# PaulMayer123/IMS-Toucan-Prosody-Variance

Measured on AMD Instinct MI355X. Metric: mel-frames/sec + vocoder RTF @24kHz, batch=32, 1/2/4/8 MI355X, higher is better.
Workload: dtype bf16

## Files before the change

ims-toucan-prosody-variance_amd/csrc/common.h:

```cpp
#pragma once
#include <hip/hip_runtime.h>
#include <stdint.h>
#include <stdio.h>

#include "../../include/toucan_tts.h"

namespace tts {

void set_error(const char* fmt, ...);

#define TTS_CHECK_ARG(cond, ...)   \
  do {                             \
    if (!(cond)) {                 \
      tts::set_error(__VA_ARGS__); \
      return TTS_E_ARG;            \
    }                              \
  } while (0)

inline int launch_status(const char* what) {
  hipError_t e = hipGetLastError();
  if (e != hipSuccess) {
    set_error("%s: %s", what, hipGetErrorString(e));
    return TTS_E_LAUNCH;
  }
// ... 2 lines not shown

inline hipError_t raise_lds_limit(const void* kernel, unsigned long long& mask) {
  int dev = 0;
  (void)hipGetDevice(&dev);
  const unsigned long long bit = 1ull << (dev & 63);
  if (mask & bit) return hipSuccess;
  int room = 160 * 1024;
  hipFuncAttributes attr;
  if (hipFuncGetAttributes(&attr, kernel) == hipSuccess) room -= (int)attr.sharedSizeBytes;
  else (void)hipGetLastError();
  const hipError_t e = hipFuncSetAttribute(kernel, hipFuncAttributeMaxDynamicSharedMemorySize, room);
  if (e == hipSuccess) mask |= bit;
  else (void)hipGetLastError();
  return e;
}

typedef float f32x16 __attribute__((ext_vector_type(16)));
typedef float f32x4 __attribute__((ext_vector_type(4)));
typedef short bf16x8 __attribute__((ext_vector_type(8)));

__device__ __forceinline__ unsigned short f32_to_bf16(float f) {
  const __bf16 b = (__bf16)f;
  return __builtin_bit_cast(unsigned short, b);
}
__device__ __forceinline__ float bf16_to_f32(unsigned short u) { return __builtin_bit_cast(float, (unsigned int)u << 16); }

typedef _Float16 f16x2 __attribute__((ext_vector_type(2)));
typedef _Float16 f16x8 __attribute__((ext_vector_type(8)));
typedef float f32x2 __attribute__((ext_vector_type(2)));
__device__ __forceinline__ unsigned short f32_to_f16(float f) { return __builtin_bit_cast(unsigned short, (_Float16)f); }
// ... 45 lines not shown
```

ims-toucan-prosody-variance_amd/csrc/pipeline.hip:

```cpp
#include <algorithm>
#include <cmath>
#include <cstdlib>
#include <cstring>
#include <string>
#include <unordered_map>
#include <utility>
#include <vector>

#include "common.h"
#include "../../include/toucan_score.h"

namespace tts {

namespace {

constexpr int ATT = 192, HEADS = 4, DK = 48;

struct Dev {
  void* p = nullptr;
  int64_t shape[4] = {0, 0, 0, 0};
  int ndim = 0, dtype = 0;
  size_t bytes = 0;
};

// ... 409 lines not shown
  b->ff_fused = find(h, p + "ff.fused");
  TTS_TRY(conv_of(h, p + "qkv", &b->qkv));
  TTS_TRY(conv_of(h, p + "out", &b->out));
  TTS_TRY(conv_of(h, p + "pos", &b->pos));
  TTS_TRY(conv_of(h, p + "pw1", &b->pw1));
  TTS_TRY(conv_of(h, p + "pw2", &b->pw2));
  TTS_TRY(fvec(h, p + "u", &b->u));
  TTS_TRY(fvec(h, p + "v", &b->v));
  TTS_TRY(fvec(h, p + "dw_w", &b->dw_w));
  TTS_TRY(fvec(h, p + "dw_b", &b->dw_b));
  return TTS_OK;
}

bool is16(const Handle* h) { return h->cfg.precision == TTS_COMPUTE_BF16 || h->cfg.precision == TTS_COMPUTE_F16; }
int bits16(const Handle* h) { return is16(h) ? 16 : 32; }

int ensure_ptabs(Handle* h, hipStream_t st) {
  const Dev* pe;
  TTS_TRY(need(h, "pe", &pe));
  const int rows = (int)pe->shape[0], pmax = (rows + 1) / 2;
  if (h->pmax == pmax && h->ptab[0]) return TTS_OK;
  TTS_TRY(hip_ok(hipStreamSynchronize(st), "position tables: sync"));
  for (int s = 0; s < 2; ++s) {
    if (h->ptab[s]) (void)hipFree(h->ptab[s]);
    TTS_TRY(hip_ok(hipMalloc(reinterpret_cast<void**>(&h->ptab[s]), (size_t)6 * rows * ATT * sizeof(float)), "position tables: hipMalloc"));
  }
  int one = rows;
  const Layout l = Layout::make(&one, 1, 1);
  for (int s = 0; s < 2; ++s)
    for (int b = 0; b < 6; ++b) {
// ... 79 lines not shown
    } else {
      TTS_TRY(tts_layernorm(x, ATT, ln, ATT, b.ln_g[3], b.ln_b[3], R, ATT, 1e-12f, st));
      TTS_TRY(conv(h, b.ff1, T2(ln, ATT), T2(hid, 1536, b16), l, st, relu));
      TTS_TRY(conv(h, b.ff2, T2(hid, 1536, b16), T2(x, ATT), l, st, half));
      TTS_TRY(tts_layernorm(x, ATT, x, ATT, b.ln_g[4], b.ln_b[4], R, ATT, 1e-12f, st));
    }
  }
  return TTS_OK;
}

size_t conformer_bytes(size_t R) { return R * (ATT * 4 * 4 + 1536 * 4 + 3 * ATT * 4) + 8 * 256; }

size_t phone_arena_bytes(size_t R, size_t B) {
  return conformer_bytes(R) + R * (100 + 3 * ATT + 6 * 256 + 16) * 4 + B * (64 + 2 * ATT + 24 * 256 + 8) * 4 + (1 << 16);
}
size_t frame_arena_bytes(size_t RF) {
  return conformer_bytes(RF) + RF * ((80 + ATT) + 2 * ATT + 3 * 80 + 2 * 256 + ATT + 160 + 4 * ATT + ATT + 8 * ATT + 64) * 4 + (64 << 20);
}
size_t vocoder_stage_bytes(size_t R, int stage, bool fused_mode, bool big) {
  static const int UPS[4] = {8, 48, 192, 384};
  const size_t ch = 256 >> stage, rows = R * UPS[stage], se = fused_mode ? 2 : 4;
  const bool fused = fused_mode && ch <= 128;
  const size_t tensors = 4 + (fused ? 0 : (big ? 3 : 1));
  return tensors * (((rows * ch * se) + 255) & ~(size_t)255) + (1 << 20);
}
size_t vocoder_arena_bytes(size_t R, int arena, bool fused_mode, bool big) {
  size_t m = arena == 1 ? R * 512 * 4 + (1 << 20) : 0;
  for (int i = arena; i < 4; i += 2) m = std::max(m, vocoder_stage_bytes(R, i, fused_mode, big));
  return m;
}
size_t with_growth_slack(size_t bytes) { return bytes + bytes / 8 + (1 << 20); }

// ... 94 lines not shown
  }
  if (dtype == 3) {
    d.p = malloc(std::max<size_t>(d.bytes, 4));
    memcpy(d.p, host, d.bytes);
  } else {
    TTS_TRY(hip_ok(hipMalloc(&d.p, std::max<size_t>(d.bytes, 256)), "tts_load_weights: hipMalloc"));
    TTS_TRY(hip_ok(hipMemcpy(d.p, host, d.bytes, hipMemcpyHostToDevice), "tts_load_weights: upload"));
  }
  h->weights[name] = d;
  return TTS_OK;
}

long long pipeline_workspace_bytes(const Handle* h, int B, int Lmax, int Tmax) {
  if (!h || B <= 0) return 0;
  const size_t RP = (size_t)B * Lmax, RF = (size_t)B * (Tmax + 1);
  size_t total = with_growth_slack(phone_arena_bytes(RP, B)) + with_growth_slack(frame_arena_bytes(RF));
  if (h->cfg.vocoder) {
    const bool fused_mode = is16(h), big = h->cfg.vocoder == 2;
    for (int a = 0; a < 2; ++a) total += with_growth_slack(vocoder_arena_bytes(RF, a, fused_mode, big));
  }
  return (long long)total;
}

long long pipeline_workspace_claimed(const Handle* h) {
  if (!h) return 0;
  return (long long)(h->phone.cap + h->frame.cap + h->voc[0].cap + h->voc[1].cap);
}

int pipeline_encoder(Handle* h, const float* text, const float* utt_emb, const int* lang_ids, const int* phone_lengths, int B,
                     hipStream_t st) {
  TTS_CHECK_ARG(h && text && phone_lengths && B > 0, "tts_encoder: bad arguments");
// ... 101 lines not shown
  const int *pb, *pe;
  TTS_TRY(bounds_of(h, h->lp, st, &pb, &pe));
  TTS_TRY(tts_prosody_control(h->text, 62, h->pitch, h->energy, h->dur, pb, pe, B, duration_scale, pitch_scale, energy_scale, pause_scale, st));
  std::vector<int> d_host(R);
  TTS_TRY(hip_ok(hipMemcpyAsync(d_host.data(), h->dur, (size_t)R * 4, hipMemcpyDeviceToHost, st), "durations to host"));
  TTS_TRY(hip_ok(hipStreamSynchronize(st), "durations to host: sync"));
  h->frames.assign(B, 0);
  for (int u = 0; u < B; ++u) {
    long long t = 0;
    for (int i = 0; i < h->lp.lengths[u]; ++i) t += d_host[h->lp.begins[u] + i];
    h->frames[u] = t > 0 ? (int)t : h->lp.lengths[u];
    if (frames_out) frames_out[u] = h->frames[u];
  }
  h->lf = Layout::make(h->frames.data(), B, 2);
  const size_t RF = h->lf.total;
  TTS_TRY(arena_reserve(h->frame, frame_arena_bytes(RF), st));
  Arena& a = h->frame;
  TTS_ALLOC(cat, a, float, RF * (80 + ATT));
  TTS_TRY(hip_ok(hipMemsetAsync(cat, 0, RF * (80 + ATT) * 4, st), "clear frame buffer"));
  TTS_ALLOC(dec, a, float, RF * ATT);
  h->cat = cat;
  h->dec = dec;
  const float *wp, *bp, *we, *be;
  TTS_TRY(fvec(h, "pitch_w", &wp));
  TTS_TRY(fvec(h, "pitch_b", &bp));
  TTS_TRY(fvec(h, "energy_w", &we));
  TTS_TRY(fvec(h, "energy_b", &be));
  const int *fb, *fe;
  TTS_TRY(bounds_of(h, h->lf, st, &fb, &fe));
  return tts_length_regulate(h->enc, ATT, h->pitch, h->energy, wp, bp, we, be, h->dur, pb, pe, fb, B, h->lf.max_len, h->lp.max_len, ATT,
                             cat + 80, 80 + ATT, dec, ATT, sqrtf((float)ATT), st);
// ... 25 lines not shown
  TTS_TRY(hip_ok(hipStreamSynchronize(st), "durations to host: sync"));
  h->frames.assign(B, 0);
  for (int u = 0; u < B; ++u) {
    long long t = 0;
    for (int i = 0; i < h->lp.lengths[u]; ++i) {
      const int d = d_host[h->lp.begins[u] + i];
      TTS_CHECK_ARG(d >= 0, "tts_teacher_forced: utterance %d, phoneme %d: negative gold duration %d", u, i, d);
      t += d;
    }
    TTS_CHECK_ARG(t <= (1 << 24), "tts_teacher_forced: utterance %d: %lld frames", u, t);
    h->frames[u] = t > 0 ? (int)t : h->lp.lengths[u];
    if (frames_out) frames_out[u] = h->frames[u];
  }
  h->lf = Layout::make(h->frames.data(), B, 2);
  const size_t RF = h->lf.total;
  TTS_TRY(arena_reserve(h->frame, frame_arena_bytes(RF), st));
  Arena& a = h->frame;
  TTS_ALLOC(cat, a, float, RF * (80 + ATT));
  TTS_TRY(hip_ok(hipMemsetAsync(cat, 0, RF * (80 + ATT) * 4, st), "clear frame buffer"));
  TTS_ALLOC(dec, a, float, RF * ATT);
  h->cat = cat;
  h->dec = dec;
  const float *wp, *bp, *we, *be;
  TTS_TRY(fvec(h, "pitch_w", &wp));
  TTS_TRY(fvec(h, "pitch_b", &bp));
  TTS_TRY(fvec(h, "energy_w", &we));
  TTS_TRY(fvec(h, "energy_b", &be));
  const int *pb, *pe, *fb, *fe;
  TTS_TRY(bounds_of(h, h->lp, st, &pb, &pe));
  TTS_TRY(bounds_of(h, h->lf, st, &fb, &fe));
  return tts_length_regulate(h->enc, ATT, h->energy, h->pitch, we, be, wp, bp, h->dur, pb, pe, fb, B, h->lf.max_len, h->lp.max_len, ATT,
// ... 55 lines not shown
  TTS_CHECK_ARG(h && h->mel == h->cat && h->cat, "tts_postflow: run tts_postnet first");
  TTS_CHECK_ARG(z_noise, "tts_postflow: z_noise is required");
  h->split_mode = 1;
  h->tab_which = 0;
  const Layout ls = h->lf.halved();
  const int RF = h->lf.total, RS = RF / 2;
  Arena& a = h->frame;
  const int b16 = bits16(h);
  ConvW gp;
  TTS_TRY(conv_of(h, "g_proj", &gp));
  TTS_ALLOC(g, a, float, (size_t)RF * ATT);
  TTS_TRY(conv(h, gp, T2(h->cat, 80 + ATT), T2(g, ATT), h->lf, st));
  TTS_ALLOC(x, a, float, (size_t)RS * 160);
  TTS_TRY(hip_ok(hipMemcpyAsync(x, z_noise, (size_t)RS * 160 * 4, hipMemcpyDeviceToDevice, st), "flow noise"));
  TTS_ALLOC(hs, a, float, (size_t)RS * 2 * ATT);
  const bool fused = is16(h) && !h->no_fused_wavenet;
  float* hs2 = nullptr;
  TileTab t64;
  if (fused) {
    hs2 = arena_alloc<float>(a, (size_t)RS * 2 * ATT);
    if (!hs2) {
      set_error("tts_postflow: workspace exhausted");
      return TTS_E_ARG;
    }
    TTS_TRY(tiles_of(h, ls, 64, st, &t64));
  }
  TTS_ALLOC(acts, a, char, (size_t)RS * ATT * (b16 / 8));
  TTS_ALLOC(cond, a, float, (size_t)RS * 8 * ATT);
  float* skip = hs + ATT;
  for (int b = 17; b >= 0; --b) {
    const std::string p = "flow." + std::to_string(b) + ".", grp = "flowgrp." + std::to_string(b / 4) + ".";
    ConvW start, end, cnd;
    TTS_TRY(conv_of(h, p + "start", &start));
    TTS_TRY(conv_of(h, p + "end", &end));
    TTS_TRY(conv_of(h, p + "cond", &cnd));
    TTS_TRY(conv(h, start, T2(x, 160), T2(hs, 2 * ATT), ls, st));
    TTS_TRY(conv(h, cnd, T2(g, 2 * ATT), T2(cond, 8 * ATT), ls, st));
    float* cur = hs;
    for (int i = 0; i < 4; ++i) {
      ConvW inl, rs;
      TTS_TRY(conv_of(h, grp + "inl." + std::to_string(i), &inl));
      TTS_TRY(conv_of(h, grp + "res_skip." + std::to_string(i), &rs));
      if (fused) {
        float* nxt = cur == hs ? hs2 : hs;
        TtsWavenetDesc w;
        memset(&w, 0, sizeof(w));
        w.hs_in = cur; w.ld_in = 2 * ATT; w.hs_out = nxt; w.ld_out = 2 * ATT;
        w.cond = cond + (size_t)i * 2 * ATT; w.ld_cond = 8 * ATT;
        w.w1 = inl.w16; w.b1 = inl.bias; w.w2 = rs.w16; w.b2 = rs.bias;
        w.cout2 = rs.cout; w.compute = inl.compute16;
        w.tiles = t64.dev; w.n_tiles = t64.n; w.tile_rows = 64;
        TTS_TRY(tts_wavenet_layer(&w, st));
        cur = nxt;
        continue;
      }
      ConvOpt oi;
      oi.preadd = cond + (size_t)i * 2 * ATT;
      oi.ld_preadd = 8 * ATT;
      TTS_TRY(conv(h, inl, T2(hs, 2 * ATT), T2(acts, ATT, b16), ls, st, oi));
      ConvOpt orr;
      orr.accumulate = true;
      TTS_TRY(conv(h, rs, T2(acts, ATT, b16), i < 3 ? T2(hs, 2 * ATT) : T2(skip, 2 * ATT), ls, st, orr));
    }
    ConvOpt oe;
    oe.aux = x + 80;
    oe.ld_aux = 160;
    oe.fp32_only = true;
// ... 374 lines not shown
```

ims-toucan-prosody-variance_amd/csrc/wavenet.hip:

```cpp
#include "common.h"

namespace tts {

namespace {
constexpr int WN_H = 192;
constexpr int WN_BM = 64;
constexpr int WN_TAPS = 5;
constexpr int WN_XP = WN_H + 8;
constexpr int WN_KS = 32;
constexpr int WN_SLAB_BYTES = (WN_KS / 8) * 384 * 16;
constexpr int WN_SLABS1 = WN_TAPS * (WN_H / WN_KS);
constexpr int WN_SLABS2 = WN_H / WN_KS;
constexpr int WN_RING = 5;
constexpr int WN_LOADS = 6;
}

template <bool F16>
__global__ __launch_bounds__(256) void wavenet_layer_kernel(const TtsWavenetDesc d) {
  extern __shared__ __attribute__((aligned(16))) unsigned char lds_raw[];
  unsigned short* xs = reinterpret_cast<unsigned short*>(lds_raw);
  unsigned char* ring = lds_raw + ((WN_BM + WN_TAPS - 1) * WN_XP * 2 + 255) / 256 * 256;
  const TtsTile tile = d.tiles[blockIdx.x];
  const int tid = threadIdx.x, lane = tid & 63, wave = tid >> 6, wm = wave >> 1, wn = wave & 1, lrow = lane & 31, lk = lane >> 5;
  const int n2 = d.cout2;
  const int units2 = (WN_KS / 8) * n2;
  const int total = WN_SLABS1 + WN_SLABS2;
  const char* w1 = reinterpret_cast<const char*>(d.w1);
  const char* w2 = reinterpret_cast<const char*>(d.w2);

  auto issue_piece = [&](int s, int i) __attribute__((always_inline)) {
    if (s >= total) return;
    const bool second = s >= WN_SLABS1;
    const int units = second ? units2 : (WN_KS / 8) * 384;
    const char* src = second ? w2 + (size_t)(s - WN_SLABS1) * units2 * 16 : w1 + (size_t)s * WN_SLAB_BYTES;
    unsigned char* dst = ring + (size_t)(s % WN_RING) * WN_SLAB_BYTES;
#ifdef WN_DIAG_NO_DMA
    if (s >= WN_RING) return;
#endif
    const int u0 = i * 256 + wave * 64;
    int u = u0 + lane;
    u = u < units ? u : units - 1;
    __builtin_amdgcn_global_load_lds((const void __attribute__((address_space(1)))*)(src + (size_t)u * 16),
                                     (void __attribute__((address_space(3)))*)(dst + (size_t)u0 * 16), 16, 0, 0);
  };
  auto issue = [&](int s) __attribute__((always_inline)) {
#pragma unroll
    for (int i = 0; i < WN_LOADS; ++i) issue_piece(s, i);
  };

#pragma unroll
  for (int i = 0; i < WN_RING - 1; ++i) issue(i);
  {
    constexpr int Q4 = WN_H / 4, ROWS = WN_BM + WN_TAPS - 1, TOTAL = ROWS * Q4, PER = 7;
    for (int base = tid; base < TOTAL; base += 256 * PER) {
      float4 v[PER];
#pragma unroll
      for (int p = 0; p < PER; ++p) {
        int e = base + p * 256;
        e = e < TOTAL ? e : TOTAL - 1;
        const int r = e / Q4, c4 = (e % Q4) * 4;
        const int gr = tile.row0 - 2 + r;
        const int grc = gr < tile.seq_begin ? tile.seq_begin : (gr >= tile.seq_end ? tile.seq_end - 1 : gr);
        v[p] = *reinterpret_cast<const float4*>(d.hs_in + (size_t)grc * d.ld_in + c4);
        if (gr != grc) v[p] = make_float4(0.f, 0.f, 0.f, 0.f);
      }
#pragma unroll
      for (int p = 0; p < PER; ++p) {
        const int e = base + p * 256;
        if (e < TOTAL) {
          const int r = e / Q4, c4 = (e % Q4) * 4;
          *reinterpret_cast<uint2*>(xs + r * WN_XP + c4) = make_uint2(pack16<F16>(v[p].x, v[p].y), pack16<F16>(v[p].z, v[p].w));
        }
      }
    }
  }
  f32x16 acc[6];
#pragma unroll
  for (int j = 0; j < 6; ++j)
#pragma unroll
    for (int r = 0; r < 16; ++r) acc[j][r] = 0.0f;

  auto wait_for = [&](int s) __attribute__((always_inline)) {
    const int behind = total - 1 - s;
    static_assert(WN_RING >= 3 && WN_RING <= 6, "one wait per number of slabs in flight below");
    if (WN_RING >= 6 && behind >= 4) asm volatile("s_waitcnt vmcnt(%0)" ::"n"(4 * WN_LOADS) : "memory");
    else if (WN_RING >= 5 && behind >= 3) asm volatile("s_waitcnt vmcnt(%0)" ::"n"(3 * WN_LOADS) : "memory");
    else if (WN_RING >= 4 && behind >= 2) asm volatile("s_waitcnt vmcnt(%0)" ::"n"(2 * WN_LOADS) : "memory");
    else if (behind >= 1) asm volatile("s_waitcnt vmcnt(%0)" ::"n"(WN_LOADS) : "memory");
    else asm volatile("s_waitcnt vmcnt(0)" ::: "memory");
    asm volatile("s_waitcnt lgkmcnt(0)" ::: "memory");
    __builtin_amdgcn_s_barrier();
  };

  for (int s = 0; s < WN_SLABS1; ++s) {
    wait_for(s);
    const int tap = s / (WN_H / WN_KS), k0 = (s % (WN_H / WN_KS)) * WN_KS;
    const unsigned short* wb = reinterpret_cast<const unsigned short*>(ring + (size_t)(s % WN_RING) * WN_SLAB_BYTES);
    bf16x8 xf[WN_KS / 16], wf[WN_KS / 16][6];
#pragma unroll
    for (int kk = 0; kk < WN_KS / 16; ++kk) {
      xf[kk] = *reinterpret_cast<const bf16x8*>(xs + (wm * 32 + lrow + tap) * WN_XP + k0 + kk * 16 + lk * 8);
#pragma unroll
      for (int j = 0; j < 6; ++j) {
        const int col = (j < 3 ? 0 : WN_H) + wn * 96 + (j % 3) * 32 + lrow;
        wf[kk][j] = *reinterpret_cast<const bf16x8*>(wb + ((size_t)(kk * 2 + lk) * 384 + col) * 8);
      }
    }
    __builtin_amdgcn_sched_barrier(0);
#ifndef WN_DIAG_NO_MFMA
#pragma unroll
    for (int kk = 0; kk < WN_KS / 16; ++kk)
#pragma unroll
      for (int j = 0; j < 6; ++j) {
        if ((kk * 6 + j) % 2 == 0) {
          issue_piece(s + WN_RING - 1, (kk * 6 + j) / 2);
          __builtin_amdgcn_sched_barrier(0);
        }
        acc[j] = mfma16<F16>(wf[kk][j], xf[kk], acc[j]);
      }
#else
    issue(s + WN_RING - 1);
    for (int j = 0; j < 6; ++j) acc[j][0] += bf16_to_f32(wf[0][j][0]) + bf16_to_f32(xf[1][1]) + bf16_to_f32(wf[1][j][2]);
#endif
    __builtin_amdgcn_sched_barrier(0);
  }
  __builtin_amdgcn_s_barrier();
  {
    const int t = wm * 32 + lrow, row = tile.row0 + t;
    const bool live = row < tile.seq_end;
    const float* cr = d.cond + (size_t)(live ? row : tile.seq_end - 1) * d.ld_cond;
#pragma unroll
    for (int j = 0; j < 3; ++j) {
#pragma unroll
      for (int rq = 0; rq < 4; ++rq) {
        const int c = wn * 96 + j * 32 + 8 * rq + 4 * lk;
        const float4 ba = *reinterpret_cast<const float4*>(d.b1 + c), bg = *reinterpret_cast<const float4*>(d.b1 + WN_H + c);
        const float4 ca = *reinterpret_cast<const float4*>(cr + c), cg = *reinterpret_cast<const float4*>(cr + WN_H + c);
        const float av[4] = {acc[j][4 * rq] + ba.x + ca.x, acc[j][4 * rq + 1] + ba.y + ca.y, acc[j][4 * rq + 2] + ba.z + ca.z, acc[j][4 * rq + 3] + ba.w + ca.w};
        const float gv[4] = {acc[j + 3][4 * rq] + bg.x + cg.x, acc[j + 3][4 * rq + 1] + bg.y + cg.y, acc[j + 3][4 * rq + 2] + bg.z + cg.z,
                             acc[j + 3][4 * rq + 3] + bg.w + cg.w};
        float v[4];
#pragma unroll
        for (int q = 0; q < 4; ++q) {
          const float th = 2.0f * __builtin_amdgcn_rcpf(1.0f + __expf(-2.0f * av[q])) - 1.0f;
          v[q] = th * __builtin_amdgcn_rcpf(1.0f + __expf(-gv[q]));
        }
        *reinterpret_cast<uint2*>(xs + t * WN_XP + c) = make_uint2(pack16<F16>(v[0], v[1]), pack16<F16>(v[2], v[3]));
      }
    }
#pragma unroll
    for (int j = 0; j < 6; ++j)
#pragma unroll
      for (int r = 0; r < 16; ++r) acc[j][r] = 0.0f;
  }
  const int half2 = n2 >> 1, nj = n2 >> 6;
  for (int s = WN_SLABS1; s < total; ++s) {
    wait_for(s);
    const int k0 = (s - WN_SLABS1) * WN_KS;
    const unsigned short* wb = reinterpret_cast<const unsigned short*>(ring + (size_t)(s % WN_RING) * WN_SLAB_BYTES);
    bf16x8 xf[WN_KS / 16], wf[WN_KS / 16][6];
#pragma unroll
    for (int kk = 0; kk < WN_KS / 16; ++kk) {
      xf[kk] = *reinterpret_cast<const bf16x8*>(xs + (wm * 32 + lrow) * WN_XP + k0 + kk * 16 + lk * 8);
#pragma unroll
      for (int j = 0; j < 6; ++j) {
        const int col = wn * half2 + (j < nj ? j : 0) * 32 + lrow;
        wf[kk][j] = *reinterpret_cast<const bf16x8*>(wb + ((size_t)(kk * 2 + lk) * n2 + col) * 8);
      }
    }
    __builtin_amdgcn_sched_barrier(0);
#pragma unroll
    for (int kk = 0; kk < WN_KS / 16; ++kk)
#pragma unroll
      for (int j = 0; j < 6; ++j) {
        if ((kk * 6 + j) % 2 == 0) {
          issue_piece(s + WN_RING - 1, (kk * 6 + j) / 2);
          __builtin_amdgcn_sched_barrier(0);
        }
        if (j < nj) acc[j] = mfma16<F16>(wf[kk][j], xf[kk], acc[j]);
      }
    __builtin_amdgcn_sched_barrier(0);
  }
  {
    const int row = tile.row0 + wm * 32 + lrow;
    if (row < tile.seq_end) {
      const int col0 = n2 == 384 ? 0 : WN_H;
      const float* ir = d.hs_in + (size_t)row * d.ld_in + col0;
      float* orow = d.hs_out + (size_t)row * d.ld_out + col0;
#pragma unroll
      for (int j = 0; j < 6; ++j) {
        if (j < nj) {
#pragma unroll
          for (int rq = 0; rq < 4; ++rq) {
            const int c = wn * half2 + j * 32 + 8 * rq + 4 * lk;
            const float4 b = *reinterpret_cast<const float4*>(d.b2 + c), x = *reinterpret_cast<const float4*>(ir + c);
            *reinterpret_cast<float4*>(orow + c) = make_float4((acc[j][4 * rq] + b.x) + x.x, (acc[j][4 * rq + 1] + b.y) + x.y,
                                                               (acc[j][4 * rq + 2] + b.z) + x.z, (acc[j][4 * rq + 3] + b.w) + x.w);
          }
        }
      }
    }
  }
}

int wavenet_layer(const TtsWavenetDesc& d, hipStream_t st) {
  TTS_CHECK_ARG(d.hs_in && d.hs_out && d.cond && d.w1 && d.b1 && d.w2 && d.b2 && d.tiles, "wavenet_layer: null pointer");
  TTS_CHECK_ARG(d.hs_in != d.hs_out, "wavenet_layer: the hidden state cannot be updated in place (the 5-tap conv reads neighbouring tiles)");
  TTS_CHECK_ARG(d.cout2 == 384 || d.cout2 == 192, "wavenet_layer: res/skip width %d (384, or 192 for the last layer)", d.cout2);
  TTS_CHECK_ARG(d.compute == TTS_COMPUTE_BF16 || d.compute == TTS_COMPUTE_F16, "wavenet_layer: 16-bit MFMA configurations only (compute %d)", d.compute);
  TTS_CHECK_ARG(d.tile_rows == WN_BM, "wavenet_layer: tile table must use %d rows, got %d", WN_BM, d.tile_rows);
  TTS_CHECK_ARG((d.ld_in & 3) == 0 && (d.ld_out & 3) == 0 && (d.ld_cond & 3) == 0 && ((uintptr_t)d.hs_in & 15) == 0 && ((uintptr_t)d.hs_out & 15) == 0 &&
                    ((uintptr_t)d.cond & 15) == 0 && ((uintptr_t)d.w1 & 15) == 0 && ((uintptr_t)d.w2 & 15) == 0 && ((uintptr_t)d.b1 & 15) == 0 &&
                    ((uintptr_t)d.b2 & 15) == 0,
                "wavenet_layer: rows and weights must be 16-byte aligned");
  if (d.n_tiles == 0) return TTS_OK;
  const size_t lds = ((size_t)(WN_BM + WN_TAPS - 1) * WN_XP * 2 + 255) / 256 * 256 + WN_RING * (size_t)WN_SLAB_BYTES;
  static unsigned long long raised[2] = {0, 0};
  const bool f16 = d.compute == TTS_COMPUTE_F16;
  const void* k = f16 ? reinterpret_cast<const void*>(wavenet_layer_kernel<true>) : reinterpret_cast<const void*>(wavenet_layer_kernel<false>);
  if (raise_lds_limit(k, raised[f16 ? 1 : 0]) != hipSuccess) {
    set_error("wavenet_layer: raising the dynamic LDS limit failed");
    return TTS_E_LAUNCH;
  }
  if (f16) hipLaunchKernelGGL(wavenet_layer_kernel<true>, dim3(d.n_tiles), dim3(256), lds, st, d);
  else hipLaunchKernelGGL(wavenet_layer_kernel<false>, dim3(d.n_tiles), dim3(256), lds, st, d);
  return launch_status("wavenet_layer");
}

}

extern "C" int tts_wavenet_layer(const TtsWavenetDesc* d, tts_stream_t stream) {
  if (!d) {
    tts::set_error("tts_wavenet_layer: null descriptor");
    return TTS_E_ARG;
  }
  return tts::wavenet_layer(*d, reinterpret_cast<hipStream_t>(stream));
}
```

Baseline: 562,300.

## Fuse flow conditioning projection into wavenet layer kernel and stream weights through registers

The postflow conditioning conv (384 -> 1536) is no longer run as a separate GEMM into a large cond buffer. Each wavenet layer kernel now loads the g rows into LDS and computes its own 384-column slice of the conditioning projection alongside the dilated conv. The weight pipeline also changes, from an LDS ring fed by global_load_lds to per-wave register prefetching with a depth-4 global_load_dwordx4 queue and a different wave-to-tile mapping. This saves a launch and the write and read of the cond tensor and shrinks the frame arena, at the cost of extra per-layer MFMA work and higher register pressure.

Measured after the change: 576,600, median of 6. 1.03x the previous value.

```diff
diff --git a/ims-toucan-prosody-variance_amd/csrc/common.h b/ims-toucan-prosody-variance_amd/csrc/common.h
--- a/ims-toucan-prosody-variance_amd/csrc/common.h
+++ b/ims-toucan-prosody-variance_amd/csrc/common.h
@@ -40,6 +40,16 @@
   else (void)hipGetLastError();
   return e;
 }
+
+struct WavenetCond {
+  const float* g;
+  int ld_g;
+  const void* wc;
+  int wc_n;
+  int col0;
+  const float* bc;
+};
+int wavenet_layer_cond(const TtsWavenetDesc& d, const WavenetCond& c, hipStream_t st);
 
 typedef float f32x16 __attribute__((ext_vector_type(16)));
 typedef float f32x4 __attribute__((ext_vector_type(4)));
diff --git a/ims-toucan-prosody-variance_amd/csrc/pipeline.hip b/ims-toucan-prosody-variance_amd/csrc/pipeline.hip
--- a/ims-toucan-prosody-variance_amd/csrc/pipeline.hip
+++ b/ims-toucan-prosody-variance_amd/csrc/pipeline.hip
@@ -447,6 +447,7 @@
 
 bool is16(const Handle* h) { return h->cfg.precision == TTS_COMPUTE_BF16 || h->cfg.precision == TTS_COMPUTE_F16; }
 int bits16(const Handle* h) { return is16(h) ? 16 : 32; }
+bool postflow_cond_buffer(const Handle* h) { return !is16(h) || h->no_fused_wavenet; }
 
 int ensure_ptabs(Handle* h, hipStream_t st) {
   const Dev* pe;
@@ -556,8 +557,8 @@
 size_t phone_arena_bytes(size_t R, size_t B) {
   return conformer_bytes(R) + R * (100 + 3 * ATT + 6 * 256 + 16) * 4 + B * (64 + 2 * ATT + 24 * 256 + 8) * 4 + (1 << 16);
 }
-size_t frame_arena_bytes(size_t RF) {
-  return conformer_bytes(RF) + RF * ((80 + ATT) + 2 * ATT + 3 * 80 + 2 * 256 + ATT + 160 + 4 * ATT + ATT + 8 * ATT + 64) * 4 + (64 << 20);
+size_t frame_arena_bytes(size_t RF, bool cond_buffer) {
+  return conformer_bytes(RF) + RF * ((80 + ATT) + 2 * ATT + 3 * 80 + 2 * 256 + ATT + 160 + 4 * ATT + ATT + (cond_buffer ? 8 * ATT : 0) + 64) * 4 + (64 << 20);
 }
 size_t vocoder_stage_bytes(size_t R, int stage, bool fused_mode, bool big) {
   static const int UPS[4] = {8, 48, 192, 384};
@@ -682,7 +683,7 @@
 long long pipeline_workspace_bytes(const Handle* h, int B, int Lmax, int Tmax) {
   if (!h || B <= 0) return 0;
   const size_t RP = (size_t)B * Lmax, RF = (size_t)B * (Tmax + 1);
-  size_t total = with_growth_slack(phone_arena_bytes(RP, B)) + with_growth_slack(frame_arena_bytes(RF));
+  size_t total = with_growth_slack(phone_arena_bytes(RP, B)) + with_growth_slack(frame_arena_bytes(RF, postflow_cond_buffer(h)));
   if (h->cfg.vocoder) {
     const bool fused_mode = is16(h), big = h->cfg.vocoder == 2;
     for (int a = 0; a < 2; ++a) total += with_growth_slack(vocoder_arena_bytes(RF, a, fused_mode, big));
@@ -814,7 +815,7 @@
   }
   h->lf = Layout::make(h->frames.data(), B, 2);
   const size_t RF = h->lf.total;
-  TTS_TRY(arena_reserve(h->frame, frame_arena_bytes(RF), st));
+  TTS_TRY(arena_reserve(h->frame, frame_arena_bytes(RF, postflow_cond_buffer(h)), st));
   Arena& a = h->frame;
   TTS_ALLOC(cat, a, float, RF * (80 + ATT));
   TTS_TRY(hip_ok(hipMemsetAsync(cat, 0, RF * (80 + ATT) * 4, st), "clear frame buffer"));
@@ -870,7 +871,7 @@
   }
   h->lf = Layout::make(h->frames.data(), B, 2);
   const size_t RF = h->lf.total;
-  TTS_TRY(arena_reserve(h->frame, frame_arena_bytes(RF), st));
+  TTS_TRY(arena_reserve(h->frame, frame_arena_bytes(RF, postflow_cond_buffer(h)), st));
   Arena& a = h->frame;
   TTS_ALLOC(cat, a, float, RF * (80 + ATT));
   TTS_TRY(hip_ok(hipMemsetAsync(cat, 0, RF * (80 + ATT) * 4, st), "clear frame buffer"));
@@ -956,7 +957,7 @@
   TTS_ALLOC(x, a, float, (size_t)RS * 160);
   TTS_TRY(hip_ok(hipMemcpyAsync(x, z_noise, (size_t)RS * 160 * 4, hipMemcpyDeviceToDevice, st), "flow noise"));
   TTS_ALLOC(hs, a, float, (size_t)RS * 2 * ATT);
-  const bool fused = is16(h) && !h->no_fused_wavenet;
+  const bool fused = !postflow_cond_buffer(h);
   float* hs2 = nullptr;
   TileTab t64;
   if (fused) {
@@ -967,9 +968,19 @@
     }
     TTS_TRY(tiles_of(h, ls, 64, st, &t64));
   }
-  TTS_ALLOC(acts, a, char, (size_t)RS * ATT * (b16 / 8));
-  TTS_ALLOC(cond, a, float, (size_t)RS * 8 * ATT);
+  char* acts = nullptr;
+  float* cond = nullptr;
+  if (!fused) {
+    acts = arena_alloc<char>(a, (size_t)RS * ATT * (b16 / 8));
+    cond = arena_alloc<float>(a, (size_t)RS * 8 * ATT);
+    if (!acts || !cond) {
+      set_error("tts_postflow: workspace exhausted");
+      return TTS_E_ARG;
+    }
+  }
   float* skip = hs + ATT;
+  double live_rows = 0;
+  for (int n : ls.lengths) live_rows += n;
   for (int b = 17; b >= 0; --b) {
     const std::string p = "flow." + std::to_string(b) + ".", grp = "flowgrp." + std::to_string(b / 4) + ".";
     ConvW start, end, cnd;
@@ -977,7 +988,7 @@
     TTS_TRY(conv_of(h, p + "end", &end));
     TTS_TRY(conv_of(h, p + "cond", &cnd));
     TTS_TRY(conv(h, start, T2(x, 160), T2(hs, 2 * ATT), ls, st));
-    TTS_TRY(conv(h, cnd, T2(g, 2 * ATT), T2(cond, 8 * ATT), ls, st));
+    if (!fused) TTS_TRY(conv(h, cnd, T2(g, 2 * ATT), T2(cond, 8 * ATT), ls, st));
     float* cur = hs;
     for (int i = 0; i < 4; ++i) {
       ConvW inl, rs;
@@ -988,11 +999,21 @@
         TtsWavenetDesc w;
         memset(&w, 0, sizeof(w));
         w.hs_in = cur; w.ld_in = 2 * ATT; w.hs_out = nxt; w.ld_out = 2 * ATT;
-        w.cond = cond + (size_t)i * 2 * ATT; w.ld_cond = 8 * ATT;
         w.w1 = inl.w16; w.b1 = inl.bias; w.w2 = rs.w16; w.b2 = rs.bias;
         w.cout2 = rs.cout; w.compute = inl.compute16;
         w.tiles = t64.dev; w.n_tiles = t64.n; w.tile_rows = 64;
-        TTS_TRY(tts_wavenet_layer(&w, st));
+        TTS_CHECK_ARG(cnd.w16 && cnd.mode == TTS_MODE_LINEAR && cnd.compute16 == inl.compute16 && cnd.cin == 2 * ATT && cnd.cin_pad == 2 * ATT && cnd.cout == 8 * ATT &&
+                          cnd.taps == 1 && cnd.wn >= 8 * ATT,
+                      "tts_postflow: %scond is not a 16-bit 1-tap 384 -> 1536 conv", p.c_str());
+        const WavenetCond wc = {g, 2 * ATT, cnd.w16, cnd.wn, i * 2 * ATT, cnd.bias};
+        ProfRec* pr = nullptr;
+        if (h->prof_on && prof_wants(h, "wavenet_layer"))
+          pr = prof_open(h, "wavenet_layer", 2.0 * live_rows * (ATT * 5 * 2 * ATT + 2 * ATT * 2 * ATT + (double)ATT * rs.cout),
+                         live_rows * 4.0 * (2 * ATT + rs.cout + 2 * ATT) + 2.0 * (5 * ATT * 2 * ATT + 2 * ATT * 2 * ATT + ATT * rs.cout),
+                         live_rows * rs.cout, st);
+        const int rc = wavenet_layer_cond(w, wc, st);
+        if (pr) (void)hipEventRecord(pr->e1, st);
+        TTS_TRY(rc);
         cur = nxt;
         continue;
       }
diff --git a/ims-toucan-prosody-variance_amd/csrc/wavenet.hip b/ims-toucan-prosody-variance_amd/csrc/wavenet.hip
--- a/ims-toucan-prosody-variance_amd/csrc/wavenet.hip
+++ b/ims-toucan-prosody-variance_amd/csrc/wavenet.hip
@@ -7,49 +7,83 @@
 constexpr int WN_BM = 64;
 constexpr int WN_TAPS = 5;
 constexpr int WN_XP = WN_H + 8;
-constexpr int WN_KS = 32;
-constexpr int WN_SLAB_BYTES = (WN_KS / 8) * 384 * 16;
-constexpr int WN_SLABS1 = WN_TAPS * (WN_H / WN_KS);
-constexpr int WN_SLABS2 = WN_H / WN_KS;
-constexpr int WN_RING = 5;
-constexpr int WN_LOADS = 6;
-}
-
-template <bool F16>
-__global__ __launch_bounds__(256) void wavenet_layer_kernel(const TtsWavenetDesc d) {
+constexpr int WN_G = 2 * WN_H;
+constexpr int WN_GP = WN_G + 8;
+constexpr int WN_STEPS1 = WN_TAPS * (WN_H / 16);
+constexpr int WN_STEPSC = WN_G / 16;
+constexpr int WN_STEPS2 = WN_H / 16;
+constexpr int WN_DEPTH = 4;
+constexpr int WN_L = 4;
+constexpr size_t WN_XS_BYTES = ((size_t)(WN_BM + WN_TAPS - 1) * WN_XP * 2 + 255) / 256 * 256;
+constexpr size_t WN_GS_BYTES = (size_t)WN_BM * WN_GP * 2;
+static_assert(WN_STEPS1 % WN_DEPTH == 0 && WN_STEPSC % WN_DEPTH == 0 && WN_STEPS2 % WN_DEPTH == 0 && (WN_H / 16) % WN_DEPTH == 0,
+              "a block of WN_DEPTH k-steps stays inside one tap and one product");
+}
+
+template <bool F16, bool FUSED>
+__global__ __launch_bounds__(256) void wavenet_layer_kernel(const TtsWavenetDesc d, const WavenetCond cd) {
   extern __shared__ __attribute__((aligned(16))) unsigned char lds_raw[];
   unsigned short* xs = reinterpret_cast<unsigned short*>(lds_raw);
-  unsigned char* ring = lds_raw + ((WN_BM + WN_TAPS - 1) * WN_XP * 2 + 255) / 256 * 256;
+  unsigned short* gs = reinterpret_cast<unsigned short*>(lds_raw + WN_XS_BYTES);
   const TtsTile tile = d.tiles[blockIdx.x];
-  const int tid = threadIdx.x, lane = tid & 63, wave = tid >> 6, wm = wave >> 1, wn = wave & 1, lrow = lane & 31, lk = lane >> 5;
+  const int tid = threadIdx.x, lane = tid & 63, lrow = lane & 31, lk = lane >> 5;
+  const int wave = __builtin_amdgcn_readfirstlane(tid >> 6);
+  const int P0 = (wave * 5 + 1) / 3, P1 = wave < 2 ? 1 : 4, fP = wave & 1, fQ = fP ^ 1;
   const int n2 = d.cout2;
-  const int units2 = (WN_KS / 8) * n2;
-  const int total = WN_SLABS1 + WN_SLABS2;
-  const char* w1 = reinterpret_cast<const char*>(d.w1);
-  const char* w2 = reinterpret_cast<const char*>(d.w2);
-
-  auto issue_piece = [&](int s, int i) __attribute__((always_inline)) {
-    if (s >= total) return;
-    const bool second = s >= WN_SLABS1;
-    const int units = second ? units2 : (WN_KS / 8) * 384;
-    const char* src = second ? w2 + (size_t)(s - WN_SLABS1) * units2 * 16 : w1 + (size_t)s * WN_SLAB_BYTES;
-    unsigned char* dst = ring + (size_t)(s % WN_RING) * WN_SLAB_BYTES;
-#ifdef WN_DIAG_NO_DMA
-    if (s >= WN_RING) return;
-#endif
-    const int u0 = i * 256 + wave * 64;
-    int u = u0 + lane;
-    u = u < units ? u : units - 1;
-    __builtin_amdgcn_global_load_lds((const void __attribute__((address_space(1)))*)(src + (size_t)u * 16),
-                                     (void __attribute__((address_space(3)))*)(dst + (size_t)u0 * 16), 16, 0, 0);
-  };
-  auto issue = [&](int s) __attribute__((always_inline)) {
-#pragma unroll
-    for (int i = 0; i < WN_LOADS; ++i) issue_piece(s, i);
-  };
-
-#pragma unroll
-  for (int i = 0; i < WN_RING - 1; ++i) issue(i);
+  const int cb0 = n2 == 384 ? 3 * wave : P0, cb1 = n2 == 384 ? 3 * wave + 1 : P1, cb2 = n2 == 384 ? 3 * wave + 2 : P1;
+
+  typedef unsigned int u32x4 __attribute__((ext_vector_type(4)));
+#define WN_GLOAD128(dst_, ptr_) asm volatile("global_load_dwordx4 %0, %1, off" : "=v"(dst_) : "v"(ptr_) : "memory")
+#define WN_WAIT_VM(n_) asm volatile("s_waitcnt vmcnt(%0)" ::"n"(n_) : "memory")
+#define WN_PIN(r_) asm volatile("" : "+v"(r_))
+  u32x4 wr[WN_DEPTH][WN_L];
+  const char *q0, *q1, *q2, *q3;
+  size_t qs;
+  auto request = [&](int slot) __attribute__((always_inline)) {
+    WN_GLOAD128(wr[slot][0], q0);
+    WN_GLOAD128(wr[slot][1], q1);
+    WN_GLOAD128(wr[slot][2], q2);
+    WN_GLOAD128(wr[slot][3], q3);
+    q0 += qs; q1 += qs; q2 += qs; q3 += qs;
+  };
+  auto arrive = [&](int slot) __attribute__((always_inline)) {
+    WN_WAIT_VM((WN_DEPTH - 1) * WN_L);
+    WN_PIN(wr[slot][0]);
+    WN_PIN(wr[slot][1]);
+    WN_PIN(wr[slot][2]);
+    WN_PIN(wr[slot][3]);
+  };
+  auto stream_pairs = [&](const void* w, int n, int col0) __attribute__((always_inline)) {
+    const char* b = reinterpret_cast<const char*>(w) + ((size_t)lk * n + col0 + lrow) * 16;
+    q0 = b + P0 * 512; q1 = q0 + WN_H * 16; q2 = b + P1 * 512; q3 = q2 + WN_H * 16;
+    qs = (size_t)n * 32;
+  };
+  auto stream_res_skip = [&]() __attribute__((always_inline)) {
+    const char* b = reinterpret_cast<const char*>(d.w2) + ((size_t)lk * n2 + lrow) * 16;
+    q0 = b + cb0 * 512; q1 = b + cb1 * 512; q2 = b + cb2 * 512; q3 = q2;
+    qs = (size_t)n2 * 32;
+  };
+  auto publish = [&]() __attribute__((always_inline)) {
+    asm volatile("s_waitcnt lgkmcnt(0)" ::: "memory");
+    __builtin_amdgcn_s_barrier();
+  };
+
+  constexpr int GQ4 = WN_G / 4, GPER = WN_BM * GQ4 / 256;
+  f32x4 gv[FUSED ? GPER : 1];
+  if constexpr (FUSED) {
+#pragma unroll
+    for (int p = 0; p < GPER; ++p) {
+      const int e = tid + p * 256, r = e / GQ4, c4 = (e % GQ4) * 4;
+      int gr = tile.row0 + r;
+      gr = gr < tile.seq_end ? gr : tile.seq_end - 1;
+      const float* gp = cd.g + (size_t)gr * cd.ld_g + c4;
+      asm volatile("global_load_dwordx4 %0, %1, off" : "=a"(gv[p]) : "v"(gp) : "memory");
+    }
+  }
+  stream_pairs(d.w1, 2 * WN_H, 0);
+#pragma unroll
+  for (int u = 0; u < WN_DEPTH; ++u) request(u);
+
   {
     constexpr int Q4 = WN_H / 4, ROWS = WN_BM + WN_TAPS - 1, TOTAL = ROWS * Q4, PER = 7;
     for (int base = tid; base < TOTAL; base += 256 * PER) {
@@ -74,158 +108,223 @@
       }
     }
   }
-  f32x16 acc[6];
+  publish();
+
+  f32x16 acc[6], accc[FUSED ? 6 : 1];
 #pragma unroll
   for (int j = 0; j < 6; ++j)
 #pragma unroll
     for (int r = 0; r < 16; ++r) acc[j][r] = 0.0f;
 
-  auto wait_for = [&](int s) __attribute__((always_inline)) {
-    const int behind = total - 1 - s;
-    static_assert(WN_RING >= 3 && WN_RING <= 6, "one wait per number of slabs in flight below");
-    if (WN_RING >= 6 && behind >= 4) asm volatile("s_waitcnt vmcnt(%0)" ::"n"(4 * WN_LOADS) : "memory");
-    else if (WN_RING >= 5 && behind >= 3) asm volatile("s_waitcnt vmcnt(%0)" ::"n"(3 * WN_LOADS) : "memory");
-    else if (WN_RING >= 4 && behind >= 2) asm volatile("s_waitcnt vmcnt(%0)" ::"n"(2 * WN_LOADS) : "memory");
-    else if (behind >= 1) asm volatile("s_waitcnt vmcnt(%0)" ::"n"(WN_LOADS) : "memory");
-    else asm volatile("s_waitcnt vmcnt(0)" ::: "memory");
-    asm volatile("s_waitcnt lgkmcnt(0)" ::: "memory");
-    __builtin_amdgcn_s_barrier();
-  };
-
-  for (int s = 0; s < WN_SLABS1; ++s) {
-    wait_for(s);
-    const int tap = s / (WN_H / WN_KS), k0 = (s % (WN_H / WN_KS)) * WN_KS;
-    const unsigned short* wb = reinterpret_cast<const unsigned short*>(ring + (size_t)(s % WN_RING) * WN_SLAB_BYTES);
-    bf16x8 xf[WN_KS / 16], wf[WN_KS / 16][6];
-#pragma unroll
-    for (int kk = 0; kk < WN_KS / 16; ++kk) {
-      xf[kk] = *reinterpret_cast<const bf16x8*>(xs + (wm * 32 + lrow + tap) * WN_XP + k0 + kk * 16 + lk * 8);
-#pragma unroll
-      for (int j = 0; j < 6; ++j) {
-        const int col = (j < 3 ? 0 : WN_H) + wn * 96 + (j % 3) * 32 + lrow;
-        wf[kk][j] = *reinterpret_cast<const bf16x8*>(wb + ((size_t)(kk * 2 + lk) * 384 + col) * 8);
-      }
-    }
-    __builtin_amdgcn_sched_barrier(0);
-#ifndef WN_DIAG_NO_MFMA
-#pragma unroll
-    for (int kk = 0; kk < WN_KS / 16; ++kk)
-#pragma unroll
-      for (int j = 0; j < 6; ++j) {
-        if ((kk * 6 + j) % 2 == 0) {
-          issue_piece(s + WN_RING - 1, (kk * 6 + j) / 2);
-          __builtin_amdgcn_sched_barrier(0);
+  auto xload = [&](bf16x8& xP, bf16x8& xQ, const unsigned short* xrow, int pitch) __attribute__((always_inline)) {
+    xP = *reinterpret_cast<const bf16x8*>(xrow + (fP * 32 + lrow) * pitch + lk * 8);
+    xQ = *reinterpret_cast<const bf16x8*>(xrow + (fQ * 32 + lrow) * pitch + lk * 8);
+  };
+  auto pair_step = [&](int slot, f32x16 (&a)[6], bf16x8& xP, bf16x8& xQ, const unsigned short* xnext, int pitch) __attribute__((always_inline)) {
+    const bf16x8 cP = xP, cQ = xQ;
+    xload(xP, xQ, xnext, pitch);
+    arrive(slot);
+    u32x4 wf[WN_L];
+#pragma unroll
+    for (int i = 0; i < WN_L; ++i) wf[i] = wr[slot][i];
+    a[0] = mfma16<F16>(__builtin_bit_cast(bf16x8, wf[0]), cP, a[0]);
+    a[1] = mfma16<F16>(__builtin_bit_cast(bf16x8, wf[0]), cQ, a[1]);
+    a[2] = mfma16<F16>(__builtin_bit_cast(bf16x8, wf[1]), cP, a[2]);
+    a[3] = mfma16<F16>(__builtin_bit_cast(bf16x8, wf[1]), cQ, a[3]);
+    a[4] = mfma16<F16>(__builtin_bit_cast(bf16x8, wf[2]), cP, a[4]);
+    a[5] = mfma16<F16>(__builtin_bit_cast(bf16x8, wf[3]), cP, a[5]);
+    request(slot);
+  };
+  bf16x8 xP, xQ;
+  auto window_at = [&](int s) __attribute__((always_inline)) {
+    s = s < WN_STEPS1 ? s : WN_STEPS1 - 1;
+    return xs + (s / (WN_H / 16)) * WN_XP + (s % (WN_H / 16)) * 16;
+  };
+
+  xload(xP, xQ, window_at(0), WN_XP);
+#pragma unroll 1
+  for (int base = 0; base < WN_STEPS1; base += WN_DEPTH) {
+    if (base == WN_STEPS1 - WN_DEPTH) {
+      if constexpr (FUSED) stream_pairs(cd.wc, cd.wc_n, cd.col0);
+      else stream_res_skip();
+    }
+#pragma unroll
+    for (int u = 0; u < WN_DEPTH; ++u) pair_step(u, acc, xP, xQ, window_at(base + u + 1), WN_XP);
+  }
+  if constexpr (FUSED) {
+#pragma unroll
+    for (int p = 0; p < GPER; ++p) {
+      asm volatile("" : "+a"(gv[p]));
+      const int e = tid + p * 256, r = e / GQ4, c4 = (e % GQ4) * 4;
+      *reinterpret_cast<uint2*>(gs + r * WN_GP + c4) = make_uint2(pack16<F16>(gv[p][0], gv[p][1]), pack16<F16>(gv[p][2], gv[p][3]));
+    }
+  }
+  publish();
+  if constexpr (FUSED) {
+#pragma unroll
+    for (int j = 0; j < 6; ++j)
+#pragma unroll
+      for (int r = 0; r < 16; ++r) accc[j][r] = 0.0f;
+    xload(xP, xQ, gs, WN_GP);
+#pragma unroll 1
+    for (int base = 0; base < WN_STEPSC; base += WN_DEPTH) {
+      if (base == WN_STEPSC - WN_DEPTH) stream_res_skip();
+#pragma unroll
+      for (int u = 0; u < WN_DEPTH; ++u) {
+        const int s1 = base + u + 1 < WN_STEPSC ? base + u + 1 : WN_STEPSC - 1;
+        pair_step(u, accc, xP, xQ, gs + s1 * 16, WN_GP);
+      }
+    }
+  }
+  {
+    auto gate = [&](const f32x16& aa, const f32x16& ag, const f32x16& ca, const f32x16& cg, int pb, int f) __attribute__((always_inline)) {
+      const int t = f * 32 + lrow, row = tile.row0 + t;
+      const float* cr = FUSED ? nullptr : d.cond + (size_t)(row < tile.seq_end ? row : tile.seq_end - 1) * d.ld_cond;
+#pragma unroll
+      for (int rq = 0; rq < 4; ++rq) {
+        const int c = pb * 32 + 8 * rq + 4 * lk;
+        const float4 ba = *reinterpret_cast<const float4*>(d.b1 + c), bg = *reinterpret_cast<const float4*>(d.b1 + WN_H + c);
+        float pa[4], pg[4];
+        if constexpr (FUSED) {
+          const float4 ea = *reinterpret_cast<const float4*>(cd.bc + cd.col0 + c), eg = *reinterpret_cast<const float4*>(cd.bc + cd.col0 + WN_H + c);
+          const float eav[4] = {ea.x, ea.y, ea.z, ea.w}, egv[4] = {eg.x, eg.y, eg.z, eg.w};
+#pragma unroll
+          for (int q = 0; q < 4; ++q) {
+            pa[q] = (ca[4 * rq + q] + eav[q]) + 0.0f;
+            pg[q] = (cg[4 * rq + q] + egv[q]) + 0.0f;
+          }
+        } else {
+          const float4 ea = *reinterpret_cast<const float4*>(cr + c), eg = *reinterpret_cast<const float4*>(cr + WN_H + c);
+          pa[0] = ea.x; pa[1] = ea.y; pa[2] = ea.z; pa[3] = ea.w;
+          pg[0] = eg.x; pg[1] = eg.y; pg[2] = eg.z; pg[3] = eg.w;
         }
-        acc[j] = mfma16<F16>(wf[kk][j], xf[kk], acc[j]);
-      }
-#else
-    issue(s + WN_RING - 1);
-    for (int j = 0; j < 6; ++j) acc[j][0] += bf16_to_f32(wf[0][j][0]) + bf16_to_f32(xf[1][1]) + bf16_to_f32(wf[1][j][2]);
-#endif
-    __builtin_amdgcn_sched_barrier(0);
-  }
-  __builtin_amdgcn_s_barrier();
-  {
-    const int t = wm * 32 + lrow, row = tile.row0 + t;
-    const bool live = row < tile.seq_end;
-    const float* cr = d.cond + (size_t)(live ? row : tile.seq_end - 1) * d.ld_cond;
-#pragma unroll
-    for (int j = 0; j < 3; ++j) {
-#pragma unroll
-      for (int rq = 0; rq < 4; ++rq) {
-        const int c = wn * 96 + j * 32 + 8 * rq + 4 * lk;
-        const float4 ba = *reinterpret_cast<const float4*>(d.b1 + c), bg = *reinterpret_cast<const float4*>(d.b1 + WN_H + c);
-        const float4 ca = *reinterpret_cast<const float4*>(cr + c), cg = *reinterpret_cast<const float4*>(cr + WN_H + c);
-        const float av[4] = {acc[j][4 * rq] + ba.x + ca.x, acc[j][4 * rq + 1] + ba.y + ca.y, acc[j][4 * rq + 2] + ba.z + ca.z, acc[j][4 * rq + 3] + ba.w + ca.w};
-        const float gv[4] = {acc[j + 3][4 * rq] + bg.x + cg.x, acc[j + 3][4 * rq + 1] + bg.y + cg.y, acc[j + 3][4 * rq + 2] + bg.z + cg.z,
-                             acc[j + 3][4 * rq + 3] + bg.w + cg.w};
+        const float bav[4] = {ba.x, ba.y, ba.z, ba.w}, bgv[4] = {bg.x, bg.y, bg.z, bg.w};
         float v[4];
 #pragma unroll
         for (int q = 0; q < 4; ++q) {
-          const float th = 2.0f * __builtin_amdgcn_rcpf(1.0f + __expf(-2.0f * av[q])) - 1.0f;
-          v[q] = th * __builtin_amdgcn_rcpf(1.0f + __expf(-gv[q]));
+          const float av = aa[4 * rq + q] + bav[q] + pa[q], gvv = ag[4 * rq + q] + bgv[q] + pg[q];
+          const float th = 2.0f * __builtin_amdgcn_rcpf(1.0f + __expf(-2.0f * av)) - 1.0f;
+          v[q] = th * __builtin_amdgcn_rcpf(1.0f + __expf(-gvv));
         }
         *reinterpret_cast<uint2*>(xs + t * WN_XP + c) = make_uint2(pack16<F16>(v[0], v[1]), pack16<F16>(v[2], v[3]));
       }
-    }
+    };
+    constexpr int CZ = FUSED ? 1 : 0;
+    gate(acc[0], acc[2], accc[0 * CZ], accc[2 * CZ], P0, fP);
+    gate(acc[1], acc[3], accc[1 * CZ], accc[3 * CZ], P0, fQ);
+    gate(acc[4], acc[5], accc[4 * CZ], accc[5 * CZ], P1, fP);
 #pragma unroll
     for (int j = 0; j < 6; ++j)
 #pragma unroll
       for (int r = 0; r < 16; ++r) acc[j][r] = 0.0f;
   }
-  const int half2 = n2 >> 1, nj = n2 >> 6;
-  for (int s = WN_SLABS1; s < total; ++s) {
-    wait_for(s);
-    const int k0 = (s - WN_SLABS1) * WN_KS;
-    const unsigned short* wb = reinterpret_cast<const unsigned short*>(ring + (size_t)(s % WN_RING) * WN_SLAB_BYTES);
-    bf16x8 xf[WN_KS / 16], wf[WN_KS / 16][6];
-#pragma unroll
-    for (int kk = 0; kk < WN_KS / 16; ++kk) {
-      xf[kk] = *reinterpret_cast<const bf16x8*>(xs + (wm * 32 + lrow) * WN_XP + k0 + kk * 16 + lk * 8);
-#pragma unroll
-      for (int j = 0; j < 6; ++j) {
-        const int col = wn * half2 + (j < nj ? j : 0) * 32 + lrow;
-        wf[kk][j] = *reinterpret_cast<const bf16x8*>(wb + ((size_t)(kk * 2 + lk) * n2 + col) * 8);
-      }
-    }
-    __builtin_amdgcn_sched_barrier(0);
-#pragma unroll
-    for (int kk = 0; kk < WN_KS / 16; ++kk)
-#pragma unroll
-      for (int j = 0; j < 6; ++j) {
-        if ((kk * 6 + j) % 2 == 0) {
-          issue_piece(s + WN_RING - 1, (kk * 6 + j) / 2);
-          __builtin_amdgcn_sched_barrier(0);
-        }
-        if (j < nj) acc[j] = mfma16<F16>(wf[kk][j], xf[kk], acc[j]);
-      }
-    __builtin_amdgcn_sched_barrier(0);
+  publish();
+  xload(xP, xQ, xs, WN_XP);
+#pragma unroll 1
+  for (int base = 0; base < WN_STEPS2; base += WN_DEPTH) {
+    if (base == WN_STEPS2 - WN_DEPTH) {
+      q0 -= qs; q1 -= qs; q2 -= qs; q3 -= qs;
+      qs = 0;
+    }
+#pragma unroll
+    for (int u = 0; u < WN_DEPTH; ++u) {
+      const bf16x8 cP = xP, cQ = xQ;
+      const int s1 = base + u + 1 < WN_STEPS2 ? base + u + 1 : WN_STEPS2 - 1;
+      xload(xP, xQ, xs + s1 * 16, WN_XP);
+      arrive(u);
+      u32x4 wf[3];
+#pragma unroll
+      for (int i = 0; i < 3; ++i) wf[i] = wr[u][i];
+      acc[0] = mfma16<F16>(__builtin_bit_cast(bf16x8, wf[0]), cP, acc[0]);
+      acc[1] = mfma16<F16>(__builtin_bit_cast(bf16x8, wf[0]), cQ, acc[1]);
+      acc[2] = mfma16<F16>(__builtin_bit_cast(bf16x8, wf[1]), cP, acc[2]);
+      if (n2 == 384) {
+        acc[3] = mfma16<F16>(__builtin_bit_cast(bf16x8, wf[1]), cQ, acc[3]);
+        acc[4] = mfma16<F16>(__builtin_bit_cast(bf16x8, wf[2]), cP, acc[4]);
+        acc[5] = mfma16<F16>(__builtin_bit_cast(bf16x8, wf[2]), cQ, acc[5]);
+      }
+      request(u);
+    }
+  }
+  WN_WAIT_VM(0);
+#pragma unroll
+  for (int u = 0; u < WN_DEPTH; ++u) {
+    WN_PIN(wr[u][0]);
+    WN_PIN(wr[u][1]);
+    WN_PIN(wr[u][2]);
+    WN_PIN(wr[u][3]);
   }
   {
-    const int row = tile.row0 + wm * 32 + lrow;
-    if (row < tile.seq_end) {
-      const int col0 = n2 == 384 ? 0 : WN_H;
+    const int col0 = n2 == 384 ? 0 : WN_H;
+    auto store_block = [&](const f32x16& a, int cb, int f) __attribute__((always_inline)) {
+      const int row = tile.row0 + f * 32 + lrow;
+      if (row >= tile.seq_end) return;
       const float* ir = d.hs_in + (size_t)row * d.ld_in + col0;
       float* orow = d.hs_out + (size_t)row * d.ld_out + col0;
 #pragma unroll
-      for (int j = 0; j < 6; ++j) {
-        if (j < nj) {
-#pragma unroll
-          for (int rq = 0; rq < 4; ++rq) {
-            const int c = wn * half2 + j * 32 + 8 * rq + 4 * lk;
-            const float4 b = *reinterpret_cast<const float4*>(d.b2 + c), x = *reinterpret_cast<const float4*>(ir + c);
-            *reinterpret_cast<float4*>(orow + c) = make_float4((acc[j][4 * rq] + b.x) + x.x, (acc[j][4 * rq + 1] + b.y) + x.y,
-                                                               (acc[j][4 * rq + 2] + b.z) + x.z, (acc[j][4 * rq + 3] + b.w) + x.w);
-          }
-        }
-      }
-    }
-  }
-}
-
-int wavenet_layer(const TtsWavenetDesc& d, hipStream_t st) {
-  TTS_CHECK_ARG(d.hs_in && d.hs_out && d.cond && d.w1 && d.b1 && d.w2 && d.b2 && d.tiles, "wavenet_layer: null pointer");
+      for (int rq = 0; rq < 4; ++rq) {
+        const int c = cb * 32 + 8 * rq + 4 * lk;
+        const float4 b = *reinterpret_cast<const float4*>(d.b2 + c), x = *reinterpret_cast<const float4*>(ir + c);
+        *reinterpret_cast<float4*>(orow + c) = make_float4((a[4 * rq] + b.x) + x.x, (a[4 * rq + 1] + b.y) + x.y, (a[4 * rq + 2] + b.z) + x.z, (a[4 * rq + 3] + b.w) + x.w);
+      }
+    };
+    store_block(acc[0], cb0, fP);
+    store_block(acc[1], cb0, fQ);
+    store_block(acc[2], cb1, fP);
+    if (n2 == 384) {
+      store_block(acc[3], cb1, fQ);
+      store_block(acc[4], cb2, fP);
+      store_block(acc[5], cb2, fQ);
+    }
+  }
+#undef WN_GLOAD128
+#undef WN_WAIT_VM
+#undef WN_PIN
+}
+
+namespace {
+int wavenet_launch(const TtsWavenetDesc& d, const WavenetCond* c, hipStream_t st) {
+  TTS_CHECK_ARG(d.hs_in && d.hs_out && d.w1 && d.b1 && d.w2 && d.b2 && d.tiles, "wavenet_layer: null pointer");
   TTS_CHECK_ARG(d.hs_in != d.hs_out, "wavenet_layer: the hidden state cannot be updated in place (the 5-tap conv reads neighbouring tiles)");
   TTS_CHECK_ARG(d.cout2 == 384 || d.cout2 == 192, "wavenet_layer: res/skip width %d (384, or 192 for the last layer)", d.cout2);
   TTS_CHECK_ARG(d.compute == TTS_COMPUTE_BF16 || d.compute == TTS_COMPUTE_F16, "wavenet_layer: 16-bit MFMA configurations only (compute %d)", d.compute);
   TTS_CHECK_ARG(d.tile_rows == WN_BM, "wavenet_layer: tile table must use %d rows, got %d", WN_BM, d.tile_rows);
-  TTS_CHECK_ARG((d.ld_in & 3) == 0 && (d.ld_out & 3) == 0 && (d.ld_cond & 3) == 0 && ((uintptr_t)d.hs_in & 15) == 0 && ((uintptr_t)d.hs_out & 15) == 0 &&
-                    ((uintptr_t)d.cond & 15) == 0 && ((uintptr_t)d.w1 & 15) == 0 && ((uintptr_t)d.w2 & 15) == 0 && ((uintptr_t)d.b1 & 15) == 0 &&
-                    ((uintptr_t)d.b2 & 15) == 0,
+  TTS_CHECK_ARG((d.ld_in & 3) == 0 && (d.ld_out & 3) == 0 && ((uintptr_t)d.hs_in & 15) == 0 && ((uintptr_t)d.hs_out & 15) == 0 && ((uintptr_t)d.w1 & 15) == 0 &&
+                    ((uintptr_t)d.w2 & 15) == 0 && ((uintptr_t)d.b1 & 15) == 0 && ((uintptr_t)d.b2 & 15) == 0,
                 "wavenet_layer: rows and weights must be 16-byte aligned");
+  if (c) {
+    TTS_CHECK_ARG(c->g && c->wc && c->bc, "wavenet_layer: null conditioning pointer");
+    TTS_CHECK_ARG(c->ld_g >= WN_G && (c->ld_g & 3) == 0 && c->col0 >= 0 && (c->col0 & 31) == 0 && c->col0 + 2 * WN_H <= c->wc_n,
+                  "wavenet_layer: conditioning columns %d .. of %d, row stride %d", c->col0, c->wc_n, c->ld_g);
+    TTS_CHECK_ARG(((uintptr_t)c->g & 15) == 0 && ((uintptr_t)c->wc & 15) == 0 && ((uintptr_t)c->bc & 15) == 0, "wavenet_layer: conditioning operands must be 16-byte aligned");
+  } else {
+    TTS_CHECK_ARG(d.cond, "wavenet_layer: null pointer");
+    TTS_CHECK_ARG((d.ld_cond & 3) == 0 && ((uintptr_t)d.cond & 15) == 0, "wavenet_layer: rows and weights must be 16-byte aligned");
+  }
   if (d.n_tiles == 0) return TTS_OK;
-  const size_t lds = ((size_t)(WN_BM + WN_TAPS - 1) * WN_XP * 2 + 255) / 256 * 256 + WN_RING * (size_t)WN_SLAB_BYTES;
-  static unsigned long long raised[2] = {0, 0};
   const bool f16 = d.compute == TTS_COMPUTE_F16;
-  const void* k = f16 ? reinterpret_cast<const void*>(wavenet_layer_kernel<true>) : reinterpret_cast<const void*>(wavenet_layer_kernel<false>);
-  if (raise_lds_limit(k, raised[f16 ? 1 : 0]) != hipSuccess) {
-    set_error("wavenet_layer: raising the dynamic LDS limit failed");
-    return TTS_E_LAUNCH;
-  }
-  if (f16) hipLaunchKernelGGL(wavenet_layer_kernel<true>, dim3(d.n_tiles), dim3(256), lds, st, d);
-  else hipLaunchKernelGGL(wavenet_layer_kernel<false>, dim3(d.n_tiles), dim3(256), lds, st, d);
+  const WavenetCond none = {nullptr, 0, nullptr, 0, 0, nullptr};
+  if (c) {
+    const size_t lds = WN_XS_BYTES + WN_GS_BYTES;
+    static unsigned long long raised[2] = {0, 0};
+    const void* k = f16 ? reinterpret_cast<const void*>(wavenet_layer_kernel<true, true>) : reinterpret_cast<const void*>(wavenet_layer_kernel<false, true>);
+    if (raise_lds_limit(k, raised[f16 ? 1 : 0]) != hipSuccess) {
+      set_error("wavenet_layer: raising the dynamic LDS limit failed");
+      return TTS_E_LAUNCH;
+    }
+    if (f16) hipLaunchKernelGGL((wavenet_layer_kernel<true, true>), dim3(d.n_tiles), dim3(256), lds, st, d, *c);
+    else hipLaunchKernelGGL((wavenet_layer_kernel<false, true>), dim3(d.n_tiles), dim3(256), lds, st, d, *c);
+  } else {
+    if (f16) hipLaunchKernelGGL((wavenet_layer_kernel<true, false>), dim3(d.n_tiles), dim3(256), WN_XS_BYTES, st, d, none);
+    else hipLaunchKernelGGL((wavenet_layer_kernel<false, false>), dim3(d.n_tiles), dim3(256), WN_XS_BYTES, st, d, none);
+  }
   return launch_status("wavenet_layer");
 }
+}
+
+int wavenet_layer(const TtsWavenetDesc& d, hipStream_t st) { return wavenet_launch(d, nullptr, st); }
+
+int wavenet_layer_cond(const TtsWavenetDesc& d, const WavenetCond& c, hipStream_t st) { return wavenet_launch(d, &c, st); }
 
 }
 
```
